# neuronika/neuronika

Measured on NVIDIA H100. Metric: forward+backward GFLOP/s, higher is better.
Workload: dtype bf16

## Files before the change

### neuronika_b200/csrc/nk_gemm_tc.cu

```cuda
#include "nk_internal.cuh"
#include "nk_ptx.cuh"

namespace {

constexpr int BLOCK_M = 128;
constexpr int BLOCK_K = 64;
constexpr int WGMMA_K = 16;
constexpr int kNumThreads = 384;
constexpr uint32_t kSmemLimit = 232448;
constexpr int kEpiCols = 64;
constexpr uint32_t kEpiStageBytes = 2 * 64 * kEpiCols * 4;

struct GemmParams {
  int64_t M, N, K;
  int64_t ldc;
  void* C;
  const void* bias;
  float alpha, beta;
  int bias_bf16;
  int bias_per_row;
  int relu;
  const void* mask;
  float* colsum;
  int num_m_blocks, num_n_blocks, num_k_blocks;
  uint32_t a_lbo, a_sbo, a_kstep;
  uint32_t b_lbo, b_sbo, b_kstep;
  int rs_world, m_rot;
  int64_t rs_rows;
  void* rs_dst[8];
  int batch, a_batched, b_batched, batch_reduce, splits;
  int64_t c_batch_stride;
  int tma_store;
};

__device__ __forceinline__ int tile_m_block(const GemmParams& p, int tile) {
  const int t = tile % p.num_m_blocks;
  if (p.rs_world == 0) return t;
  const int owner = (t + p.m_rot) % p.rs_world;
  return owner * (p.num_m_blocks / p.rs_world) + t / p.rs_world;
}

constexpr int kGroupM = 16;
__device__ __forceinline__ void tile_coords(const GemmParams& p, int tile, int& m_blk, int& n_blk) {
  if (p.rs_world) {
    m_blk = tile_m_block(p, tile);
    n_blk = tile / p.num_m_blocks;
    return;
  }
  const int group_size = kGroupM * p.num_n_blocks;
  const int group = tile / group_size, in_group = tile - group * group_size;
  const int first_m = group * kGroupM;
  const int gm = min(p.num_m_blocks - first_m, kGroupM);
  m_blk = first_m + in_group % gm;
  n_blk = in_group / gm;
}

template <int BLOCK_N>
struct Cfg {
  static constexpr uint32_t A_BYTES = BLOCK_M * BLOCK_K * 2;
  static constexpr uint32_t B_BYTES = BLOCK_N * BLOCK_K * 2;
  static constexpr uint32_t STAGE_BYTES = A_BYTES + B_BYTES;
  static constexpr int kStagesMax = (kSmemLimit - 2048 - kEpiStageBytes) / STAGE_BYTES;
  static constexpr int kStages = kStagesMax > 8 ? 8 : kStagesMax;
  static constexpr uint32_t SMEM_BYTES = kStages * STAGE_BYTES + 2048 + kEpiStageBytes;
};

__device__ __forceinline__ void scale_and_bias(const GemmParams& p, int64_t row, int64_t col0, const uint32_t* r, bool full,
                                               float* v) {
#pragma unroll
  for (int j = 0; j < 32; ++j) v[j] = __fmul_rn(p.alpha, __uint_as_float(r[j]));
  if (p.bias && p.bias_per_row) {
    const float b = p.bias_bf16 ? __bfloat162float(static_cast<const __nv_bfloat16*>(p.bias)[row]) : static_cast<const float*>(p.bias)[row];
#pragma unroll
    for (int j = 0; j < 32; ++j) v[j] += b;
  } else if (p.bias) {
    if (full && (reinterpret_cast<uintptr_t>(p.bias) & 15) == 0) {
      if (p.bias_bf16) {
        const uint4* bp = reinterpret_cast<const uint4*>(static_cast<const __nv_bfloat16*>(p.bias) + col0);
#pragma unroll
        for (int q = 0; q < 4; ++q) {
          const uint4 w = __ldg(bp + q);
          const uint32_t ww[4] = {w.x, w.y, w.z, w.w};
#pragma unroll
          for (int i = 0; i < 4; ++i) {
            v[q * 8 + 2 * i] += __uint_as_float(ww[i] << 16);
            v[q * 8 + 2 * i + 1] += __uint_as_float(ww[i] & 0xffff0000u);
          }
        }
      } else {
        const float4* bp = reinterpret_cast<const float4*>(static_cast<const float*>(p.bias) + col0);
#pragma unroll
        for (int q = 0; q < 8; ++q) {
          const float4 w = __ldg(bp + q);
          v[q * 4] += w.x, v[q * 4 + 1] += w.y, v[q * 4 + 2] += w.z, v[q * 4 + 3] += w.w;
        }
      }
    } else {
#pragma unroll
      for (int j = 0; j < 32; ++j)
        if (col0 + j < p.N)
          v[j] += p.bias_bf16 ? __bfloat162float(static_cast<const __nv_bfloat16*>(p.bias)[col0 + j])
                              : static_cast<const float*>(p.bias)[col0 + j];
    }
  }
}

template <typename TC>
__device__ __forceinline__ void epilogue_colsum_chunk32(const GemmParams& p, int64_t row, int64_t col0, const uint32_t* r,
                                                        int lane, bool vec_ok) {
  float v[32];
  const bool live = row < p.M;
  const TC* mrow = (p.mask && live) ? static_cast<const TC*>(p.mask) + row * p.ldc + col0 : nullptr;
  const bool full = col0 + 32 <= p.N;
#pragma unroll
  for (int j = 0; j < 32; ++j) v[j] = (live && col0 + j < p.N) ? p.alpha * __uint_as_float(r[j]) : 0.f;
  if (mrow) {
    if (full && vec_ok) {
      constexpr int V = 16 / sizeof(TC);
#pragma unroll
      for (int q = 0; q < 32 / V; ++q) {
        NkVec<TC> mk;
        mk.load(mrow + q * V);
#pragma unroll
        for (int i = 0; i < V; ++i) v[q * V + i] = mk.get(i) > 0.f ? v[q * V + i] : 0.f;
      }
    } else {
#pragma unroll
      for (int j = 0; j < 32; ++j)
        if (col0 + j < p.N) v[j] = nk_to_f32<TC>(mrow[j]) > 0.f ? v[j] : 0.f;
    }
  }
#pragma unroll
  for (int j = 0; j < 32; ++j) v[j] = nk_to_f32<TC>(nk_from_f32<TC>(v[j]));
#pragma unroll
  for (int off = 16; off >= 1; off >>= 1) {
    const bool upper = (lane & off) != 0;
#pragma unroll
    for (int i = 0; i < off; ++i) {
      const float send = upper ? v[i] : v[i + off];
      const float keep = upper ? v[i + off] : v[i];
      v[i] = keep + __shfl_xor_sync(0xffffffffu, send, off);
    }
  }
  if (col0 + lane < p.N) atomicAdd(p.colsum + col0 + lane, v[0]);
}

template <typename TC>
__device__ __forceinline__ void epilogue_store_chunk32(const GemmParams& p, int64_t row, int64_t col0, const uint32_t* r,
                                                       int ncols, bool vec_ok, int64_t c_off = 0, bool atomic = false) {
  TC* crow = static_cast<TC*>(p.C) + c_off + row * p.ldc + col0;
  if (atomic) {
    if constexpr (sizeof(TC) == 4) {
#pragma unroll
      for (int j = 0; j < 32; ++j)
        if (j < ncols && col0 + j < p.N) atomicAdd(reinterpret_cast<float*>(crow) + j, p.alpha * __uint_as_float(r[j]));
    }
    return;
  }
  if (p.rs_world) {
    const int owner = int(row / p.rs_rows);
    crow = static_cast<TC*>(p.rs_dst[owner]) + (row - owner * p.rs_rows) * p.ldc + col0;
  }
  float v[32];
  const bool full = (col0 + 32 <= p.N) && ncols == 32;
  scale_and_bias(p, row, col0, r, full, v);
  const TC* mrow = p.mask ? static_cast<const TC*>(p.mask) + row * p.ldc + col0 : nullptr;
  if (full && vec_ok) {
    constexpr int V = 16 / sizeof(TC);
    if (mrow) {
#pragma unroll
      for (int q = 0; q < 32 / V; ++q) {
        NkVec<TC> mk;
        mk.load(mrow + q * V);
#pragma unroll
        for (int i = 0; i < V; ++i) v[q * V + i] = mk.get(i) > 0.f ? v[q * V + i] : 0.f;
      }
    }
    if (p.beta != 0.f) {
#pragma unroll
      for (int q = 0; q < 32 / V; ++q) {
        NkVec<TC> c;
        c.load(crow + q * V);
#pragma unroll
        for (int i = 0; i < V; ++i) v[q * V + i] += p.beta * c.get(i);
      }
    }
    if (p.relu) {
#pragma unroll
      for (int j = 0; j < 32; ++j) v[j] = v[j] > 0.f ? v[j] : 0.f;
    }
#pragma unroll
    for (int q = 0; q < 32 / V; ++q) {
      NkVec<TC> o;
#pragma unroll
      for (int i = 0; i < V; ++i) o.set(i, v[q * V + i]);
      o.store(crow + q * V);
    }
  } else {
#pragma unroll
    for (int j = 0; j < 32; ++j) {
      if (j < ncols && col0 + j < p.N) {
        float x = v[j];
        if (mrow) x = nk_to_f32<TC>(mrow[j]) > 0.f ? x : 0.f;
        if (p.beta != 0.f) x += p.beta * nk_to_f32<TC>(crow[j]);
        if (p.relu) x = x > 0.f ? x : 0.f;
        crow[j] = nk_from_f32<TC>(x);
      }
    }
  }
}

__device__ __forceinline__ int epi_index(int row, int col) {
  return row * kEpiCols + ((((col >> 2) ^ (row & 7))) << 2) + (col & 3);
}

__device__ __forceinline__ float col_bias(const GemmParams& p, int64_t col) {
  if (col >= p.N) return 0.f;
  return p.bias_bf16 ? __bfloat162float(static_cast<const __nv_bfloat16*>(p.bias)[col]) : static_cast<const float*>(p.bias)[col];
}

__device__ __forceinline__ float epi_value(const GemmParams& p, float acc, float bias) {
  float v = __fmul_rn(p.alpha, acc);
  if (p.bias) v += bias;
  return p.relu ? (v > 0.f ? v : 0.f) : v;
}

template <int BLOCK_N, bool A_MN, bool B_MN, typename TC, bool BATCH = false>
__global__ void __launch_bounds__(kNumThreads, 1)
gemm_tc_kernel(const __grid_constant__ CUtensorMap tmap_a, const __grid_constant__ CUtensorMap tmap_b,
               const __grid_constant__ CUtensorMap tmap_c, const GemmParams p) {
  using C_ = Cfg<BLOCK_N>;
  constexpr int kStages = C_::kStages;
  constexpr int kStoreCols = 128 / int(sizeof(TC));
  constexpr bool kTmaStore = !BATCH && BLOCK_N % kStoreCols == 0;
  static_assert(2 * 2 * 64 * 128 <= kEpiStageBytes, "staging buffers");
  extern __shared__ uint8_t smem_raw[];
  const uint32_t smem_base = (ptx::smem_u32(smem_raw) + 1023u) & ~1023u;
  const uint32_t smem_a0 = smem_base;
  const uint32_t smem_b0 = smem_base + kStages * C_::A_BYTES;
  const uint32_t bar_base = smem_base + kStages * C_::STAGE_BYTES;
  auto full_bar = [&](int s) { return bar_base + 8u * s; };
  auto empty_bar = [&](int s) { return bar_base + 8u * (kStages + s); };
  const uint32_t epi_stage = bar_base + 1024;
  float* epi = reinterpret_cast<float*>(smem_raw + (epi_stage - ptx::smem_u32(smem_raw)));

  const int wg = threadIdx.x >> 7;
  const int lane = threadIdx.x & 31;

  if (threadIdx.x == 0) {
    ptx::prefetch_tmap(&tmap_a);
    ptx::prefetch_tmap(&tmap_b);
    if (kTmaStore && p.tma_store) ptx::prefetch_tmap(&tmap_c);
    for (int s = 0; s < kStages; ++s) {
      ptx::mbar_init(full_bar(s), 1);
      ptx::mbar_init(empty_bar(s), 2);
    }
    ptx::fence_barrier_init();
  }
  __syncthreads();

  const int tiles_mn = p.num_m_blocks * p.num_n_blocks;
  const int num_tiles = BATCH ? tiles_mn * (p.batch_reduce ? p.splits : p.batch) : tiles_mn;
  auto batch_range = [&](int outer, int& b0, int& b1) {
    if (!p.batch_reduce) {
      b0 = outer, b1 = outer + 1;
    } else {
      const int per = (p.batch + p.splits - 1) / p.splits;
      b0 = outer * per;
      b1 = min(p.batch, b0 + per);
    }
  };

  if (wg == 0) {
    ptx::setmaxnreg_dec<40>();
    if (threadIdx.x == 0) {
      int stage = 0;
      uint32_t phase = 0;
      for (int tile = blockIdx.x; tile < num_tiles; tile += gridDim.x) {
        int m_blk, n_blk, b0 = 0, b1 = 1;
        tile_coords(p, BATCH ? tile % tiles_mn : tile, m_blk, n_blk);
        if (BATCH) batch_range(tile / tiles_mn, b0, b1);
        const int m0 = m_blk * BLOCK_M, n0 = n_blk * BLOCK_N;
        for (int bb = b0; bb < b1; ++bb)
        for (int kb = 0; kb < p.num_k_blocks; ++kb) {
          ptx::mbar_wait_spin(empty_bar(stage), phase ^ 1u);
          ptx::mbar_expect_tx(full_bar(stage), C_::STAGE_BYTES);
          const int k0 = kb * BLOCK_K;
          const uint32_t sa = smem_a0 + stage * C_::A_BYTES;
          const uint32_t sb = smem_b0 + stage * C_::B_BYTES;
          if (A_MN) {
#pragma unroll
            for (int c = 0; c < BLOCK_M / 64; ++c) {
              if (BATCH && p.a_batched)
                ptx::tma_load_3d(sa + c * (64 * BLOCK_K * 2), &tmap_a, full_bar(stage), m0 + c * 64, k0, bb);
              else
                ptx::tma_load_2d(sa + c * (64 * BLOCK_K * 2), &tmap_a, full_bar(stage), m0 + c * 64, k0);
            }
          } else {
            if (BATCH && p.a_batched)
              ptx::tma_load_3d(sa, &tmap_a, full_bar(stage), k0, m0, bb);
            else
              ptx::tma_load_2d(sa, &tmap_a, full_bar(stage), k0, m0);
          }
          if (B_MN) {
#pragma unroll
            for (int c = 0; c < BLOCK_N / 64; ++c) {
              if (BATCH && p.b_batched)
                ptx::tma_load_3d(sb + c * (64 * BLOCK_K * 2), &tmap_b, full_bar(stage), n0 + c * 64, k0, bb);
              else
                ptx::tma_load_2d(sb + c * (64 * BLOCK_K * 2), &tmap_b, full_bar(stage), n0 + c * 64, k0);
            }
          } else {
            if (BATCH && p.b_batched)
              ptx::tma_load_3d(sb, &tmap_b, full_bar(stage), k0, n0, bb);
            else
              ptx::tma_load_2d(sb, &tmap_b, full_bar(stage), k0, n0);
          }
          if (++stage == kStages) {
            stage = 0;
            phase ^= 1u;
          }
        }
      }
    }
    return;
  }

  ptx::setmaxnreg_inc<232>();
  const int cw = wg - 1;
  const int t = threadIdx.x & 127;
  const int warp = t >> 5;
  const bool vec_ok = ((p.ldc * int64_t(sizeof(TC))) % 16 == 0) && ((reinterpret_cast<uintptr_t>(p.C) & 15) == 0) &&
                      ((reinterpret_cast<uintptr_t>(p.mask) & 15) == 0);
  float* stg = epi + cw * (64 * kEpiCols);
  const uint32_t a_off = uint32_t(cw) * (64 * BLOCK_K * 2);
  float acc[BLOCK_N / 2];
  int stage = 0;
  uint32_t phase = 0;
  uint32_t store_buf = 0;
  for (int tile = blockIdx.x; tile < num_tiles; tile += gridDim.x) {
    int m_blk, n_blk;
    tile_coords(p, BATCH ? tile % tiles_mn : tile, m_blk, n_blk);
    int k_total = p.num_k_blocks;
    if (BATCH) {
      int b0, b1;
      batch_range(tile / tiles_mn, b0, b1);
      k_total *= (b1 - b0);
    }
    int prev_stage = 0;
    for (int kb = 0; kb < k_total; ++kb) {
      ptx::mbar_wait_spin(full_bar(stage), phase);
      const uint64_t adesc = ptx::make_smem_desc_sw128(smem_a0 + stage * C_::A_BYTES + a_off, p.a_lbo, p.a_sbo);
      const uint64_t bdesc = ptx::make_smem_desc_sw128(smem_b0 + stage * C_::B_BYTES, p.b_lbo, p.b_sbo);
      ptx::fence_regs(acc);
      ptx::wgmma_fence();
#pragma unroll
      for (int k = 0; k < BLOCK_K / WGMMA_K; ++k)
        ptx::Wgmma<BLOCK_N>::template mma<int(A_MN), int(B_MN)>(acc, adesc + uint64_t((k * p.a_kstep) >> 4),
                                                                 bdesc + uint64_t((k * p.b_kstep) >> 4), (kb | k) != 0 ? 1u : 0u);
      ptx::wgmma_commit();
      ptx::wgmma_wait<1>();
      ptx::fence_regs(acc);
      if (kb > 0 && t == 0) ptx::mbar_arrive(empty_bar(prev_stage));
      prev_stage = stage;
      if (++stage == kStages) {
        stage = 0;
        phase ^= 1u;
      }
    }
    ptx::wgmma_wait<0>();
    ptx::fence_regs(acc);
    if (t == 0) ptx::mbar_arrive(empty_bar(prev_stage));

    if constexpr (kTmaStore) {
      if (p.tma_store) {
        const int fr = warp * 16 + (lane >> 2);
        const int q = lane & 3;
        const int row0 = m_blk * BLOCK_M + cw * 64;
        const uint32_t stg0 = epi_stage + uint32_t(cw) * (2 * 64 * 128);
#pragma unroll
        for (int ch = 0; ch < BLOCK_N / kStoreCols; ++ch) {
          const uint32_t buf = stg0 + store_buf * (64 * 128);
          if (t == 0) ptx::tma_store_wait_read<1>();
          ptx::named_barrier(1 + cw, 128);
          const int64_t col0 = int64_t(n_blk) * BLOCK_N + ch * kStoreCols;
#pragma unroll
          for (int jj = 0; jj < kStoreCols / 8; ++jj) {
            const int j = (ch * (kStoreCols / 8) + jj) * 4;
            const int64_t col = col0 + jj * 8 + 2 * q;
            float b0 = 0.f, b1 = 0.f;
            if (p.bias) b0 = col_bias(p, col), b1 = col_bias(p, col + 1);
            const float v0 = epi_value(p, acc[j], b0), v1 = epi_value(p, acc[j + 1], b1);
            const float v2 = epi_value(p, acc[j + 2], b0), v3 = epi_value(p, acc[j + 3], b1);
            if constexpr (sizeof(TC) == 2) {
              const uint32_t off = fr * 128 + ((jj ^ (fr & 7)) << 4) + 4 * q;
              const __nv_bfloat162 lo = __floats2bfloat162_rn(v0, v1), hi = __floats2bfloat162_rn(v2, v3);
              ptx::st_shared_b32(buf + off, *reinterpret_cast<const uint32_t*>(&lo));
              ptx::st_shared_b32(buf + off + 8 * 128, *reinterpret_cast<const uint32_t*>(&hi));
            } else {
              const uint32_t off = fr * 128 + (((2 * jj + (q >> 1)) ^ (fr & 7)) << 4) + (q & 1) * 8;
              ptx::st_shared_v2_f32(buf + off, v0, v1);
              ptx::st_shared_v2_f32(buf + off + 8 * 128, v2, v3);
            }
          }
          ptx::fence_proxy_async();
          ptx::named_barrier(1 + cw, 128);
          if (t == 0) {
            if (row0 < p.M && col0 < p.N) ptx::tma_store_2d(&tmap_c, buf, int(col0), row0);
            ptx::tma_store_commit();
          }
          store_buf ^= 1u;
        }
        continue;
      }
    }

    const int64_t c_off = (BATCH && !p.batch_reduce) ? int64_t(tile / tiles_mn) * p.c_batch_stride : 0;
    const bool atomic = BATCH && p.batch_reduce;
    const int fr = warp * 16 + (lane >> 2);
    const int fc = (lane & 3) * 2;
    const int half = warp >> 1;
    const int rloc = (warp & 1) * 32 + lane;
    const int64_t row = int64_t(m_blk) * BLOCK_M + cw * 64 + rloc;
    constexpr int kChunks = (BLOCK_N + kEpiCols - 1) / kEpiCols;
#pragma unroll
    for (int ch = 0; ch < kChunks; ++ch) {
      constexpr int kFullBlocks = kEpiCols / 8;
      ptx::named_barrier(1 + cw, 128);
#pragma unroll
      for (int nb = 0; nb < kFullBlocks; ++nb) {
        if (ch * kFullBlocks + nb < BLOCK_N / 8) {
          const int j = (ch * kFullBlocks + nb) * 4;
          *reinterpret_cast<float2*>(stg + epi_index(fr, nb * 8 + fc)) = make_float2(acc[j], acc[j + 1]);
          *reinterpret_cast<float2*>(stg + epi_index(fr + 8, nb * 8 + fc)) = make_float2(acc[j + 2], acc[j + 3]);
        }
      }
      ptx::named_barrier(1 + cw, 128);
      const int chunk_cols = BLOCK_N - ch * kEpiCols < kEpiCols ? BLOCK_N - ch * kEpiCols : kEpiCols;
      if (!vec_ok && !p.colsum && !p.mask && !p.rs_world) {
        const int64_t col_base = int64_t(n_blk) * BLOCK_N + ch * kEpiCols;
        for (int rr = 0; rr < 16; ++rr) {
          const int srow = warp * 16 + rr;
          const int64_t grow = int64_t(m_blk) * BLOCK_M + cw * 64 + srow;
          if (grow >= p.M) break;
          float rb = 0.f;
          if (p.bias && p.bias_per_row)
            rb = p.bias_bf16 ? __bfloat162float(static_cast<const __nv_bfloat16*>(p.bias)[grow]) : static_cast<const float*>(p.bias)[grow];
          for (int c = lane; c < chunk_cols; c += 32) {
            const int64_t col = col_base + c;
            if (col >= p.N) break;
            float v = __fmul_rn(p.alpha, stg[epi_index(srow, c)]);
            TC* cp = static_cast<TC*>(p.C) + c_off + grow * p.ldc + col;
            if (atomic) {
              if constexpr (sizeof(TC) == 4) atomicAdd(reinterpret_cast<float*>(cp), v);
              continue;
            }
            if (p.bias) {
              v += p.bias_per_row ? rb
                                  : (p.bias_bf16 ? __bfloat162float(static_cast<const __nv_bfloat16*>(p.bias)[col])
                                                 : static_cast<const float*>(p.bias)[col]);
            }
            if (p.beta != 0.f) v += p.beta * nk_to_f32<TC>(*cp);
            if (p.relu) v = v > 0.f ? v : 0.f;
            *cp = nk_from_f32<TC>(v);
          }
        }
        continue;
      }
      const int ncols = min(32, chunk_cols - half * 32);
      if (ncols > 0) {
        uint32_t r[32];
#pragma unroll
        for (int q = 0; q < 8; ++q) {
          float4 v = make_float4(0.f, 0.f, 0.f, 0.f);
          if (q * 4 < ncols) v = *reinterpret_cast<const float4*>(stg + epi_index(rloc, half * 32 + q * 4));
          r[4 * q] = __float_as_uint(v.x), r[4 * q + 1] = __float_as_uint(v.y);
          r[4 * q + 2] = __float_as_uint(v.z), r[4 * q + 3] = __float_as_uint(v.w);
        }
        const int64_t col0 = int64_t(n_blk) * BLOCK_N + ch * kEpiCols + half * 32;
        if (p.colsum && col0 < p.N) epilogue_colsum_chunk32<TC>(p, row, col0, r, lane, vec_ok);
        if (row < p.M && col0 < p.N) epilogue_store_chunk32<TC>(p, row, col0, r, ncols, vec_ok, c_off, atomic);
      }
    }
  }
  if (kTmaStore && p.tma_store && t == 0) ptx::tma_store_wait<0>();
}

typedef CUresult (*EncodeTiledFn)(CUtensorMap*, CUtensorMapDataType, cuuint32_t, void*, const cuuint64_t*,
                                  const cuuint64_t*, const cuuint32_t*, const cuuint32_t*, CUtensorMapInterleave,
                                  CUtensorMapSwizzle, CUtensorMapL2promotion, CUtensorMapFloatOOBfill);

int make_tmap_2d(nk_ctx* ctx, CUtensorMap* tm, const void* base, int64_t rows, int64_t cols, int64_t ld,
                 uint32_t box_cols, uint32_t box_rows, int dtype = NK_BF16) {
  if (!ctx->encode_tiled) return nk_set_error(ctx, NK_ERR_CUDA, "cuTensorMapEncodeTiled unavailable");
  cuuint64_t dims[2] = {(cuuint64_t)cols, (cuuint64_t)rows};
  cuuint64_t strides[1] = {(cuuint64_t)ld * nk_dtype_size(dtype)};
  cuuint32_t box[2] = {box_cols, box_rows};
  cuuint32_t estr[2] = {1, 1};
  CUresult r = reinterpret_cast<EncodeTiledFn>(ctx->encode_tiled)(
      tm, dtype == NK_BF16 ? CU_TENSOR_MAP_DATA_TYPE_BFLOAT16 : CU_TENSOR_MAP_DATA_TYPE_FLOAT32, 2,
      const_cast<void*>(base), dims, strides, box, estr,
      CU_TENSOR_MAP_INTERLEAVE_NONE, CU_TENSOR_MAP_SWIZZLE_128B, CU_TENSOR_MAP_L2_PROMOTION_L2_256B,
      CU_TENSOR_MAP_FLOAT_OOB_FILL_NONE);
  if (r != CUDA_SUCCESS)
    return nk_set_error(ctx, NK_ERR_CUDA, "cuTensorMapEncodeTiled failed (%d) rows=%lld cols=%lld ld=%lld", (int)r,
                        (long long)rows, (long long)cols, (long long)ld);
  return NK_OK;
}

template <int BLOCK_N, bool A_MN, bool B_MN, typename TC, bool BATCH = false>
int launch_cfg(nk_ctx* ctx, const CUtensorMap& ta, const CUtensorMap& tb, const CUtensorMap& tc, GemmParams& p) {
  using C_ = Cfg<BLOCK_N>;
  auto kern = gemm_tc_kernel<BLOCK_N, A_MN, B_MN, TC, BATCH>;
  static bool attr_done[64] = {};
  if (!attr_done[ctx->device & 63]) {
    static_assert(C_::SMEM_BYTES <= kSmemLimit, "shared memory budget");
    NK_CUDA(ctx, cudaFuncSetAttribute(kern, cudaFuncAttributeMaxDynamicSharedMemorySize, (int)C_::SMEM_BYTES));
    attr_done[ctx->device & 63] = true;
  }
  p.num_n_blocks = int((p.N + BLOCK_N - 1) / BLOCK_N);
  int num_tiles = p.num_m_blocks * p.num_n_blocks;
  if (BATCH) {
    if (p.batch_reduce) {
      int want = (ctx->sm_count + num_tiles - 1) / num_tiles;
      if (want > p.batch) want = p.batch;
      const int per = (p.batch + want - 1) / want;
      p.splits = (p.batch + per - 1) / per;
      num_tiles *= p.splits;
    } else {
      num_tiles *= p.batch;
    }
  }
  const int units = ctx->sm_count;
  const int waves = (num_tiles + units - 1) / units;
  const int grid = (num_tiles + waves - 1) / waves;
  const size_t smem = C_::SMEM_BYTES;
  if (p.rs_world) {
    if (BLOCK_N != 256 || sizeof(TC) != 4 || p.N % 4 != 0)
      return nk_set_error(ctx, NK_ERR_UNSUPPORTED, "wgmma gemm: reduce-scatter epilogue needs 128x256 tiles, f32, N %% 4 == 0");
  }
  kern<<<grid, kNumThreads, smem, ctx->stream>>>(ta, tb, tc, p);
  ctx->launches++;
  cudaError_t le = cudaGetLastError();
  if (le != cudaSuccess)
    return nk_set_error(ctx, NK_ERR_CUDA, "launch of gemm_wgmma failed: %s (M=%lld N=%lld K=%lld BLOCK_N=%d grid=%d smem=%zu "
                        "a_mn=%d b_mn=%d out=%s)", cudaGetErrorString(le), (long long)p.M, (long long)p.N, (long long)p.K,
                        BLOCK_N, grid, smem, int(A_MN), int(B_MN), sizeof(TC) == 4 ? "f32" : "bf16");
  return NK_OK;
}

template <bool A_MN, bool B_MN, typename TC>
int launch_bn(nk_ctx* ctx, int block_n, const CUtensorMap& ta, const CUtensorMap& tb, const CUtensorMap& tc, GemmParams& p) {
  switch (block_n) {
    case 256: return launch_cfg<256, A_MN, B_MN, TC>(ctx, ta, tb, tc, p);
    case 128: return launch_cfg<128, A_MN, B_MN, TC>(ctx, ta, tb, tc, p);
    case 64: return launch_cfg<64, A_MN, B_MN, TC>(ctx, ta, tb, tc, p);
    default:
      if (!B_MN) {
        if (block_n == 32) return launch_cfg<32, A_MN, false, TC>(ctx, ta, tb, tc, p);
        if (block_n == 16) return launch_cfg<16, A_MN, false, TC>(ctx, ta, tb, tc, p);
      }
      return nk_set_error(ctx, NK_ERR_UNSUPPORTED, "wgmma gemm: unsupported BLOCK_N %d", block_n);
  }
}

}

bool nk_gemm_wgmma_supported(int transA, int transB, int64_t M, int64_t N, int64_t K, const void* A, int64_t lda,
                             const void* B, int64_t ldb) {
  (void)transA;
  (void)transB;
  if (M <= 0 || N <= 0 || K <= 0) return false;
  if ((reinterpret_cast<uintptr_t>(A) & 15) || (reinterpret_cast<uintptr_t>(B) & 15)) return false;
  if ((lda * 2) % 16 != 0 || (ldb * 2) % 16 != 0) return false;
  if (M > (int64_t(1) << 30) || N > (int64_t(1) << 30) || K > (int64_t(1) << 30)) return false;
  return true;
}

int nk_gemm_wgmma(nk_ctx* ctx, int transA, int transB, int64_t M, int64_t N, int64_t K, float alpha, const void* A,
                  int64_t lda, const void* B, int64_t ldb, float beta, void* C, int64_t ldc, int c_dtype,
                  const void* bias, int bias_dtype, int relu, const void* mask, float* colsum) {
  if (!nk_gemm_wgmma_supported(transA, transB, M, N, K, A, lda, B, ldb)) return NK_ERR_UNSUPPORTED;
  if (colsum && (N <= 16 || beta != 0.f)) return NK_ERR_UNSUPPORTED;
  const bool a_mn = transA != 0;
  const bool b_mn = transB == 0;
  int block_n = 256;
  if (N <= 16 && !b_mn)
    block_n = 16;
  else if (N <= 32 && !b_mn)
    block_n = 32;
  else if (N <= 64)
    block_n = 64;
  else if (N <= 128)
    block_n = 128;

  GemmParams p;
  p.M = M;
  p.N = N;
  p.K = K;
  p.ldc = ldc;
  p.C = C;
  p.bias = bias;
  p.alpha = alpha;
  p.beta = beta;
  p.bias_bf16 = bias_dtype == NK_BF16;
  p.bias_per_row = 0;
  p.relu = relu;
  p.mask = mask;
  p.colsum = colsum;
  p.batch = 1, p.a_batched = p.b_batched = p.batch_reduce = 0, p.splits = 1, p.c_batch_stride = 0;
  p.num_m_blocks = int((M + BLOCK_M - 1) / BLOCK_M);
  p.num_n_blocks = 0;
  p.num_k_blocks = int((K + BLOCK_K - 1) / BLOCK_K);
  p.rs_world = 0;
  p.m_rot = 0;
  p.rs_rows = M;
  for (int i = 0; i < 8; ++i) p.rs_dst[i] = nullptr;
  if (ctx->rs_world > 1) {
    if (M % (int64_t(ctx->rs_world) * BLOCK_M) != 0 || beta != 0.f || c_dtype != NK_F32)
      return nk_set_error(ctx, NK_ERR_INVALID_ARG, "wgmma gemm: reduce-scatter epilogue needs M %% (world*128) == 0, "
                          "beta == 0 and f32 output");
    p.rs_world = ctx->rs_world;
    p.rs_rows = M / ctx->rs_world;
    p.m_rot = ctx->rs_rank;
    for (int i = 0; i < ctx->rs_world; ++i) p.rs_dst[i] = ctx->rs_dst[i];
  }
  p.a_lbo = a_mn ? BLOCK_K * 128 : 16;
  p.a_sbo = 1024;
  p.a_kstep = a_mn ? WGMMA_K * 128 : WGMMA_K * 2;
  p.b_lbo = b_mn ? BLOCK_K * 128 : 16;
  p.b_sbo = 1024;
  p.b_kstep = b_mn ? WGMMA_K * 128 : WGMMA_K * 2;

  CUtensorMap ta, tb;
  int rc;
  if (a_mn)
    rc = make_tmap_2d(ctx, &ta, A, K, M, lda, 64, BLOCK_K);
  else
    rc = make_tmap_2d(ctx, &ta, A, M, K, lda, BLOCK_K, BLOCK_M);
  if (rc) return rc;
  if (b_mn)
    rc = make_tmap_2d(ctx, &tb, B, K, N, ldb, 64, BLOCK_K);
  else
    rc = make_tmap_2d(ctx, &tb, B, N, K, ldb, BLOCK_K, (uint32_t)block_n);
  if (rc) return rc;
  const int64_t c_size = int64_t(nk_dtype_size(c_dtype));
  CUtensorMap tc;
  memset(&tc, 0, sizeof(tc));
  p.tma_store = beta == 0.f && !mask && !colsum && !p.rs_world && (block_n * c_size) % 128 == 0 &&
                (reinterpret_cast<uintptr_t>(C) & 15) == 0 && (ldc * c_size) % 16 == 0 && (N * c_size) % 16 == 0;
  if (p.tma_store) {
    rc = make_tmap_2d(ctx, &tc, C, M, N, ldc, uint32_t(128 / c_size), 64, c_dtype);
    if (rc) return rc;
  }

  static const char* names[2][2][5] = {
      {{"wgmma_nt_128x256", "wgmma_nt_128x128", "wgmma_nt_128x64", "wgmma_nt_128x32", "wgmma_nt_128x16"},
       {"wgmma_nn_128x256", "wgmma_nn_128x128", "wgmma_nn_128x64", "", ""}},
      {{"wgmma_tt_128x256", "wgmma_tt_128x128", "wgmma_tt_128x64", "wgmma_tt_128x32", "wgmma_tt_128x16"},
       {"wgmma_tn_128x256", "wgmma_tn_128x128", "wgmma_tn_128x64", "", ""}}};
  const int bi = block_n == 256 ? 0 : block_n == 128 ? 1 : block_n == 64 ? 2 : block_n == 32 ? 3 : 4;
  ctx->last_gemm_kernel = names[a_mn][b_mn][bi];

#define NK_TC(AM, BM_)                                                              \
  (c_dtype == NK_BF16 ? launch_bn<AM, BM_, __nv_bfloat16>(ctx, block_n, ta, tb, tc, p) \
                      : launch_bn<AM, BM_, float>(ctx, block_n, ta, tb, tc, p))
  if (!a_mn && !b_mn) return NK_TC(false, false);
  if (!a_mn && b_mn) return NK_TC(false, true);
  if (a_mn && !b_mn) return NK_TC(true, false);
  return NK_TC(true, true);
#undef NK_TC
}

static int make_tmap_3d(nk_ctx* ctx, CUtensorMap* tm, const void* base, int64_t rows, int64_t cols, int64_t ld, int64_t batch,
                        int64_t batch_stride, uint32_t box_cols, uint32_t box_rows) {
  if (!ctx->encode_tiled) return nk_set_error(ctx, NK_ERR_CUDA, "cuTensorMapEncodeTiled unavailable");
  cuuint64_t dims[3] = {(cuuint64_t)cols, (cuuint64_t)rows, (cuuint64_t)batch};
  cuuint64_t strides[2] = {(cuuint64_t)ld * 2, (cuuint64_t)batch_stride * 2};
  cuuint32_t box[3] = {box_cols, box_rows, 1};
  cuuint32_t estr[3] = {1, 1, 1};
  CUresult r = reinterpret_cast<EncodeTiledFn>(ctx->encode_tiled)(
      tm, CU_TENSOR_MAP_DATA_TYPE_BFLOAT16, 3, const_cast<void*>(base), dims, strides, box, estr,
      CU_TENSOR_MAP_INTERLEAVE_NONE, CU_TENSOR_MAP_SWIZZLE_128B, CU_TENSOR_MAP_L2_PROMOTION_L2_256B,
      CU_TENSOR_MAP_FLOAT_OOB_FILL_NONE);
  if (r != CUDA_SUCCESS)
    return nk_set_error(ctx, NK_ERR_CUDA, "cuTensorMapEncodeTiled (3-d) failed (%d) rows=%lld cols=%lld ld=%lld batch=%lld stride=%lld",
                        (int)r, (long long)rows, (long long)cols, (long long)ld, (long long)batch, (long long)batch_stride);
  return NK_OK;
}

int nk_gemm_wgmma_batched(nk_ctx* ctx, int transA, int transB, int64_t M, int64_t N, int64_t K, float alpha, const void* A,
                            int64_t lda, int64_t strideA, const void* B, int64_t ldb, int64_t strideB, void* C, int64_t ldc,
                            int64_t strideC, int64_t batch, int c_dtype, const void* row_bias, int bias_dtype, int relu,
                            int reduce) {
  if (!nk_gemm_wgmma_supported(transA, transB, M, N, K, A, lda, B, ldb)) return NK_ERR_UNSUPPORTED;
  if (batch < 1 || batch > (int64_t(1) << 30) || (strideA * 2) % 16 != 0 || (strideB * 2) % 16 != 0) return NK_ERR_UNSUPPORTED;
  if (reduce && c_dtype != NK_F32) return NK_ERR_UNSUPPORTED;
  const bool a_mn = transA != 0, b_mn = transB == 0;
  int block_n = N <= 64 ? 64 : (N <= 128 ? 128 : 256);
  GemmParams p;
  p.M = M, p.N = N, p.K = K, p.ldc = ldc, p.C = C;
  p.bias = row_bias, p.bias_bf16 = bias_dtype == NK_BF16, p.bias_per_row = 1;
  p.alpha = alpha, p.beta = 0.f, p.relu = relu, p.mask = nullptr, p.colsum = nullptr;
  p.num_m_blocks = int((M + BLOCK_M - 1) / BLOCK_M);
  p.num_n_blocks = 0;
  p.num_k_blocks = int((K + BLOCK_K - 1) / BLOCK_K);
  p.rs_world = 0, p.m_rot = 0, p.rs_rows = M;
  for (int i = 0; i < 8; ++i) p.rs_dst[i] = nullptr;
  p.batch = int(batch), p.a_batched = strideA != 0, p.b_batched = strideB != 0, p.batch_reduce = reduce ? 1 : 0, p.splits = 1;
  p.c_batch_stride = strideC;
  p.tma_store = 0;
  p.a_lbo = a_mn ? BLOCK_K * 128 : 16, p.a_sbo = 1024, p.a_kstep = a_mn ? WGMMA_K * 128 : WGMMA_K * 2;
  p.b_lbo = b_mn ? BLOCK_K * 128 : 16, p.b_sbo = 1024, p.b_kstep = b_mn ? WGMMA_K * 128 : WGMMA_K * 2;
  CUtensorMap ta, tb;
  int rc;
  if (p.a_batched)
    rc = a_mn ? make_tmap_3d(ctx, &ta, A, K, M, lda, batch, strideA, 64, BLOCK_K)
              : make_tmap_3d(ctx, &ta, A, M, K, lda, batch, strideA, BLOCK_K, BLOCK_M);
  else
    rc = a_mn ? make_tmap_2d(ctx, &ta, A, K, M, lda, 64, BLOCK_K) : make_tmap_2d(ctx, &ta, A, M, K, lda, BLOCK_K, BLOCK_M);
  if (rc) return rc;
  if (p.b_batched)
    rc = b_mn ? make_tmap_3d(ctx, &tb, B, K, N, ldb, batch, strideB, 64, BLOCK_K)
              : make_tmap_3d(ctx, &tb, B, N, K, ldb, batch, strideB, BLOCK_K, (uint32_t)block_n);
  else
    rc = b_mn ? make_tmap_2d(ctx, &tb, B, K, N, ldb, 64, BLOCK_K) : make_tmap_2d(ctx, &tb, B, N, K, ldb, BLOCK_K, (uint32_t)block_n);
  if (rc) return rc;
  CUtensorMap tc;
  memset(&tc, 0, sizeof(tc));
  ctx->last_gemm_kernel = "wgmma_batched";
#define NK_TCB(BN, AM, BM_)                                                                          \
  (c_dtype == NK_BF16 ? launch_cfg<BN, AM, BM_, __nv_bfloat16, true>(ctx, ta, tb, tc, p)              \
                      : launch_cfg<BN, AM, BM_, float, true>(ctx, ta, tb, tc, p))
#define NK_TCB_BN(AM, BM_) (block_n == 256 ? NK_TCB(256, AM, BM_) : block_n == 128 ? NK_TCB(128, AM, BM_) : NK_TCB(64, AM, BM_))
  if (!a_mn && !b_mn) return NK_TCB_BN(false, false);
  if (!a_mn && b_mn) return NK_TCB_BN(false, true);
  if (a_mn && b_mn) return NK_TCB_BN(true, true);
  return nk_set_error(ctx, NK_ERR_UNSUPPORTED, "batched gemm: the TT form is not instantiated");
#undef NK_TCB_BN
#undef NK_TCB
}

extern "C" {

int nk_gemm_bias_act(nk_ctx* ctx, int transA, int transB, int64_t M, int64_t N, int64_t K, float alpha,
                     const void* A, int64_t lda, const void* B, int64_t ldb, float beta, void* C, int64_t ldc,
                     int ab_dtype, int c_dtype, const void* bias, int bias_dtype, int relu) {
  if (!ctx) return NK_ERR_INVALID_ARG;
  NK_REQUIRE(ctx, nk_dtype_ok(ab_dtype) && nk_dtype_ok(c_dtype), "nk_gemm: bad dtype");
  NK_REQUIRE(ctx, M >= 0 && N >= 0 && K >= 0, "nk_gemm: negative dimension");
  if (M == 0 || N == 0) return NK_OK;
  NK_REQUIRE(ctx, C != nullptr && (K == 0 || (A && B)), "nk_gemm: NULL pointer");
  NK_REQUIRE(ctx, lda >= (transA ? M : K) && ldb >= (transB ? K : N) && ldc >= N,
             "nk_gemm: leading dimension too small (lda=%lld ldb=%lld ldc=%lld for M=%lld N=%lld K=%lld tA=%d tB=%d)",
             (long long)lda, (long long)ldb, (long long)ldc, (long long)M, (long long)N, (long long)K, transA, transB);
  NK_REQUIRE(ctx, !bias || nk_dtype_ok(bias_dtype), "nk_gemm: bad bias dtype");
  const bool want_tc = ab_dtype == NK_BF16 && ctx->gemm_engine != NK_GEMM_SIMT && K > 0;
  if (want_tc) {
    int rc = nk_gemm_wgmma(ctx, transA, transB, M, N, K, alpha, A, lda, B, ldb, beta, C, ldc, c_dtype, bias,
                             bias_dtype, relu, nullptr, nullptr);
    if (rc != NK_ERR_UNSUPPORTED) return rc;
    if (ctx->gemm_engine == NK_GEMM_TC)
      return nk_set_error(ctx, NK_ERR_UNSUPPORTED,
                          "nk_gemm: tensor-core engine forced but operands are not TMA-addressable "
                          "(16-byte aligned base, leading dimension multiple of 8 elements)");
  } else if (ctx->gemm_engine == NK_GEMM_TC) {
    return nk_set_error(ctx, NK_ERR_UNSUPPORTED, "nk_gemm: tensor-core engine forced but operands are not bf16");
  }
  return nk_gemm_simt(ctx, transA, transB, M, N, K, alpha, A, lda, B, ldb, beta, C, ldc, ab_dtype, c_dtype, bias,
                      bias_dtype, relu);
}

int nk_gemm_relu_bwd_colsum(nk_ctx* ctx, int transA, int transB, int64_t M, int64_t N, int64_t K, const void* A, int64_t lda,
                            const void* B, int64_t ldb, float beta, void* C, int64_t ldc, int ab_dtype, int c_dtype,
                            const void* relu_operand, float* colsum) {
  if (!ctx) return NK_ERR_INVALID_ARG;
  NK_REQUIRE(ctx, nk_dtype_ok(ab_dtype) && nk_dtype_ok(c_dtype), "nk_gemm_relu_bwd: bad dtype");
  NK_REQUIRE(ctx, M >= 0 && N >= 0 && K > 0, "nk_gemm_relu_bwd: bad dimension");
  if (M == 0 || N == 0) return NK_OK;
  NK_REQUIRE(ctx, A && B && C && relu_operand, "nk_gemm_relu_bwd: NULL pointer");
  NK_REQUIRE(ctx, lda >= (transA ? M : K) && ldb >= (transB ? K : N) && ldc >= N, "nk_gemm_relu_bwd: leading dimension too small");
  NK_REQUIRE(ctx, !colsum || beta == 0.f, "nk_gemm_relu_bwd_colsum: the column sums are those of the product (beta must be 0)");
  if (ab_dtype == NK_BF16 && ctx->gemm_engine != NK_GEMM_SIMT) {
    int rc = nk_gemm_wgmma(ctx, transA, transB, M, N, K, 1.f, A, lda, B, ldb, beta, C, ldc, c_dtype, nullptr, NK_F32, 0,
                             relu_operand, colsum);
    if (rc != NK_ERR_UNSUPPORTED) return rc;
  }
  if (!transA && !transB) {
    int rc = nk_gemm_simt_small_k_masked(ctx, M, N, K, A, lda, B, ldb, beta, C, ldc, ab_dtype, c_dtype, relu_operand, colsum);
    if (rc != NK_ERR_UNSUPPORTED) return rc;
  }
  if (colsum) return NK_ERR_UNSUPPORTED;
  void* tmp = nullptr;
  int rc = nk_alloc_uninit(ctx, size_t(M) * size_t(N) * nk_dtype_size(c_dtype), &tmp);
  if (rc) return rc;
  rc = nk_gemm_simt(ctx, transA, transB, M, N, K, 1.f, A, lda, B, ldb, 0.f, tmp, N, ab_dtype, c_dtype, nullptr, NK_F32, 0);
  if (rc == NK_OK) {
    if (ldc == N) {
      rc = nk_relu_bwd(ctx, C, relu_operand, tmp, size_t(M) * size_t(N), c_dtype, beta);
    } else {
      rc = nk_set_error(ctx, NK_ERR_UNSUPPORTED, "nk_gemm_relu_bwd: strided output needs the tensor-core engine");
    }
  }
  nk_free(ctx, tmp);
  return rc;
}

int nk_gemm_relu_bwd(nk_ctx* ctx, int transA, int transB, int64_t M, int64_t N, int64_t K, const void* A, int64_t lda,
                     const void* B, int64_t ldb, float beta, void* C, int64_t ldc, int ab_dtype, int c_dtype,
                     const void* relu_operand) {
  return nk_gemm_relu_bwd_colsum(ctx, transA, transB, M, N, K, A, lda, B, ldb, beta, C, ldc, ab_dtype, c_dtype, relu_operand,
                                 nullptr);
}

int nk_gemm(nk_ctx* ctx, int transA, int transB, int64_t M, int64_t N, int64_t K, float alpha, const void* A,
            int64_t lda, const void* B, int64_t ldb, float beta, void* C, int64_t ldc, int ab_dtype, int c_dtype) {
  return nk_gemm_bias_act(ctx, transA, transB, M, N, K, alpha, A, lda, B, ldb, beta, C, ldc, ab_dtype, c_dtype,
                          nullptr, NK_F32, 0);
}

}
```

Measured before the change: 570,300.

## Offload TMA epilogue stores to a dedicated producer-warp thread with mbarriers

Moves TMA store issue from the consumer warpgroups to a dedicated thread in the producer warpgroup. Staging buffers are handed off through per-warpgroup staged/free mbarriers, which replace the named barriers and the store-read waits on the math warps. Bias is now prefetched once per tile into registers before the final wgmma wait and distributed by warp shuffles. This should shorten the epilogue stall so math warps start the next tile sooner, but it adds mbarrier handshake complexity and extra barrier slots in shared memory.

```diff
diff --git a/neuronika_b200/csrc/nk_gemm_tc.cu b/neuronika_b200/csrc/nk_gemm_tc.cu
--- a/neuronika_b200/csrc/nk_gemm_tc.cu
+++ b/neuronika_b200/csrc/nk_gemm_tc.cu
@@ -241,6 +241,8 @@
   const uint32_t bar_base = smem_base + kStages * C_::STAGE_BYTES;
   auto full_bar = [&](int s) { return bar_base + 8u * s; };
   auto empty_bar = [&](int s) { return bar_base + 8u * (kStages + s); };
+  auto staged_bar = [&](int cw, uint32_t b) { return bar_base + 8u * (2 * kStages + 2 * cw + b); };
+  auto free_bar = [&](int cw, uint32_t b) { return bar_base + 8u * (2 * kStages + 4 + 2 * cw + b); };
   const uint32_t epi_stage = bar_base + 1024;
   float* epi = reinterpret_cast<float*>(smem_raw + (epi_stage - ptx::smem_u32(smem_raw)));
 
@@ -255,6 +257,11 @@
       ptx::mbar_init(full_bar(s), 1);
       ptx::mbar_init(empty_bar(s), 2);
     }
+    for (int cw = 0; cw < 2; ++cw)
+      for (uint32_t b = 0; b < 2; ++b) {
+        ptx::mbar_init(staged_bar(cw, b), 4);
+        ptx::mbar_init(free_bar(cw, b), 1);
+      }
     ptx::fence_barrier_init();
   }
   __syncthreads();
@@ -322,6 +329,26 @@
           }
         }
       }
+    } else if (kTmaStore && p.tma_store && threadIdx.x == 32) {
+      uint32_t n = 0;
+      for (int tile = blockIdx.x; tile < num_tiles; tile += gridDim.x) {
+        int m_blk, n_blk;
+        tile_coords(p, tile, m_blk, n_blk);
+        for (int ch = 0; ch < BLOCK_N / kStoreCols; ++ch, ++n) {
+          const uint32_t b = n & 1u;
+          const int col0 = n_blk * BLOCK_N + ch * kStoreCols;
+          for (int cw = 0; cw < 2; ++cw) {
+            ptx::mbar_wait_spin(staged_bar(cw, b), (n >> 1) & 1u);
+            const int row0 = m_blk * BLOCK_M + cw * 64;
+            if (row0 < p.M && col0 < p.N)
+              ptx::tma_store_2d(&tmap_c, epi_stage + uint32_t(cw) * (2 * 64 * 128) + b * (64 * 128), col0, row0);
+            ptx::tma_store_commit();
+            ptx::tma_store_wait_read<2>();
+            if (n > 0) ptx::mbar_arrive(free_bar(cw, b ^ 1u));
+          }
+        }
+      }
+      ptx::tma_store_wait<0>();
     }
     return;
   }
@@ -337,7 +364,7 @@
   float acc[BLOCK_N / 2];
   int stage = 0;
   uint32_t phase = 0;
-  uint32_t store_buf = 0;
+  uint32_t store_n = 0;
   for (int tile = blockIdx.x; tile < num_tiles; tile += gridDim.x) {
     int m_blk, n_blk;
     tile_coords(p, BATCH ? tile % tiles_mn : tile, m_blk, n_blk);
@@ -368,6 +395,11 @@
         phase ^= 1u;
       }
     }
+    float bias_w[(BLOCK_N + 31) / 32];
+    if (kTmaStore && p.tma_store && p.bias) {
+#pragma unroll
+      for (int i = 0; i < (BLOCK_N + 31) / 32; ++i) bias_w[i] = col_bias(p, int64_t(n_blk) * BLOCK_N + 32 * i + lane);
+    }
     ptx::wgmma_wait<0>();
     ptx::fence_regs(acc);
     if (t == 0) ptx::mbar_arrive(empty_bar(prev_stage));
@@ -376,20 +408,21 @@
       if (p.tma_store) {
         const int fr = warp * 16 + (lane >> 2);
         const int q = lane & 3;
-        const int row0 = m_blk * BLOCK_M + cw * 64;
         const uint32_t stg0 = epi_stage + uint32_t(cw) * (2 * 64 * 128);
 #pragma unroll
-        for (int ch = 0; ch < BLOCK_N / kStoreCols; ++ch) {
-          const uint32_t buf = stg0 + store_buf * (64 * 128);
-          if (t == 0) ptx::tma_store_wait_read<1>();
-          ptx::named_barrier(1 + cw, 128);
-          const int64_t col0 = int64_t(n_blk) * BLOCK_N + ch * kStoreCols;
+        for (int ch = 0; ch < BLOCK_N / kStoreCols; ++ch, ++store_n) {
+          const uint32_t b = store_n & 1u;
+          const uint32_t buf = stg0 + b * (64 * 128);
+          ptx::mbar_wait_spin(free_bar(cw, b), ((store_n >> 1) & 1u) ^ 1u);
 #pragma unroll
           for (int jj = 0; jj < kStoreCols / 8; ++jj) {
             const int j = (ch * (kStoreCols / 8) + jj) * 4;
-            const int64_t col = col0 + jj * 8 + 2 * q;
+            const int c = ch * kStoreCols + jj * 8;
             float b0 = 0.f, b1 = 0.f;
-            if (p.bias) b0 = col_bias(p, col), b1 = col_bias(p, col + 1);
+            if (p.bias) {
+              b0 = __shfl_sync(0xffffffffu, bias_w[c / 32], c % 32 + 2 * q);
+              b1 = __shfl_sync(0xffffffffu, bias_w[c / 32], c % 32 + 2 * q + 1);
+            }
             const float v0 = epi_value(p, acc[j], b0), v1 = epi_value(p, acc[j + 1], b1);
             const float v2 = epi_value(p, acc[j + 2], b0), v3 = epi_value(p, acc[j + 3], b1);
             if constexpr (sizeof(TC) == 2) {
@@ -404,12 +437,8 @@
             }
           }
           ptx::fence_proxy_async();
-          ptx::named_barrier(1 + cw, 128);
-          if (t == 0) {
-            if (row0 < p.M && col0 < p.N) ptx::tma_store_2d(&tmap_c, buf, int(col0), row0);
-            ptx::tma_store_commit();
-          }
-          store_buf ^= 1u;
+          __syncwarp();
+          if (lane == 0) ptx::mbar_arrive(staged_bar(cw, b));
         }
         continue;
       }
@@ -483,7 +512,6 @@
       }
     }
   }
-  if (kTmaStore && p.tma_store && t == 0) ptx::tma_store_wait<0>();
 }
 
 typedef CUresult (*EncodeTiledFn)(CUtensorMap*, CUtensorMapDataType, cuuint32_t, void*, const cuuint64_t*,
```

After: 580,200 (median of 6 runs). +1.7%, better.
